# roatienza/efficientspeech

Measured on AMD Instinct MI355X. Metric: mel-frames/sec (whole node), full Phoneme2Mel forward, higher is better.
Workload: dtype f32 (weight GEMMs: fp32 operands split into 2 f16 pieces (22 significand bits, weights pre-scaled 2^8), 3 f16-MFMA products, fp32 accumulate)

## Files before the change

efficientspeech_amd/csrc/esmi_dev.h:

```cpp
#pragma once
#include "wavesim_shim.h"

namespace esmi {

__device__ __forceinline__ bf16x3 split_bf16x3(const f32x4& x0, const f32x4& x1) {
    unsigned h[8], m[8], l[8];
#pragma unroll
    for (int j = 0; j < 8; ++j) {
        const float x = j < 4 ? x0[j & 3] : x1[j & 3];
        h[j] = __builtin_bit_cast(unsigned, x) & 0xFFFF0000u;
        const float r1 = x - __builtin_bit_cast(float, h[j]);
        m[j] = __builtin_bit_cast(unsigned, r1) & 0xFFFF0000u;
        const float r2 = r1 - __builtin_bit_cast(float, m[j]);
        l[j] = __builtin_bit_cast(unsigned, r2);
    }
    bf16x3 o;
#pragma unroll
    for (int j = 0; j < 4; ++j) {
        o.hi[j] = pack_hi16(h[2 * j], h[2 * j + 1]);
        o.mid[j] = pack_hi16(m[2 * j], m[2 * j + 1]);
        o.lo[j] = pack_hi16(l[2 * j], l[2 * j + 1]);
    }
    return o;
}
__device__ __forceinline__ f32x16 mfma32_split(const bf16x3& a, const u32x4& bh, const u32x4& bm, const u32x4& bl, f32x16 c) {
    c = mfma32_bf16(a.hi, bh, c);
    c = mfma32_bf16(a.hi, bm, c);
    c = mfma32_bf16(a.mid, bh, c);
    c = mfma32_bf16(a.mid, bm, c);
    c = mfma32_bf16(a.hi, bl, c);
    c = mfma32_bf16(a.lo, bh, c);
    return c;
}
__device__ __forceinline__ f32x16 mfma32_split_wx(const u32x4& bh, const u32x4& bm, const u32x4& bl, const bf16x3& a, f32x16 c) {
    c = mfma32_bf16(bh, a.hi, c);
    c = mfma32_bf16(bm, a.hi, c);
    c = mfma32_bf16(bh, a.mid, c);
    c = mfma32_bf16(bm, a.mid, c);
    c = mfma32_bf16(bl, a.hi, c);
    c = mfma32_bf16(bh, a.lo, c);
    return c;
}

__device__ __forceinline__ f16x2p split_f16x2(const f32x4& x0, const f32x4& x1) {
    f16x2p o;
#pragma unroll
    for (int j = 0; j < 4; ++j) {
        const float a = j < 2 ? x0[2 * j] : x1[2 * j - 4], b = j < 2 ? x0[2 * j + 1] : x1[2 * j - 3];
        unsigned h1, h2;
        split_f16_pair(a, b, h1, h2);
        o.h1[j] = h1;
        o.h2[j] = h2;
    }
    return o;
}
__device__ __forceinline__ f32x16 mfma32_split2(const f16x2p& a, const u32x4& b1, const u32x4& b2, f32x16 c) {
    c = mfma32_f16(a.h2, b1, c);
    c = mfma32_f16(a.h1, b2, c);
    c = mfma32_f16(a.h1, b1, c);
    return c;
}
__device__ __forceinline__ f32x16 mfma32_split2_wx(const u32x4& b1, const u32x4& b2, const f16x2p& a, f32x16 c) {
    c = mfma32_f16(b1, a.h2, c);
    c = mfma32_f16(b2, a.h1, c);
    c = mfma32_f16(b1, a.h1, c);
    return c;
}

__device__ __forceinline__ float row_sum32(float v) {
    v += dpp_f<0xB1>(v);
    v += dpp_f<0x4E>(v);
    v += dpp_f<0x141>(v);
    v += dpp_f<0x140>(v);
    v += swz_xor16_f(v);
    return v;
}
__device__ __forceinline__ float row_sum16(float v) {
    v += dpp_f<0xB1>(v);
    v += dpp_f<0x4E>(v);
    v += dpp_f<0x141>(v);
    v += dpp_f<0x140>(v);
    return v;
}
template <int N>
__device__ __forceinline__ float row_sum_n(float v) {
    v += dpp_f<0xB1>(v);
    v += dpp_f<0x4E>(v);
    if (N >= 8) v += dpp_f<0x141>(v);
    if (N >= 16) v += dpp_f<0x140>(v);
    return v;
}
__device__ __forceinline__ float row_max32(float v) {
    v = fmaxf(v, dpp_f<0xB1>(v));
    v = fmaxf(v, dpp_f<0x4E>(v));
    v = fmaxf(v, dpp_f<0x141>(v));
    v = fmaxf(v, dpp_f<0x140>(v));
    v = fmaxf(v, swz_xor16_f(v));
    return v;
}

__device__ __forceinline__ float gelu_fast_f32(float x) {
    const float z = fabsf(x) * 0.70710678118654752440f;
    const float t = rcp_fast_f32(fmaf(0.3275911f, z, 1.0f));
    float pl = fmaf(1.061405429f, t, -1.453152027f);
    pl = fmaf(pl, t, 1.421413741f);
    pl = fmaf(pl, t, -0.284496736f);
    pl = fmaf(pl, t, 0.254829592f);
    const float erf_abs = 1.0f - pl * t * exp_fast_f32(-z * z);
    return 0.5f * x * (1.0f + copysignf(erf_abs, x));
}
__device__ __forceinline__ float ident_f32(float x) { return x; }
__device__ __forceinline__ float gelu_erf_f32(float x) {
    return 0.5f * x * (1.0f + erff(x * 0.70710678118654752440f));
}
enum Act { ACT_NONE = 0, ACT_RELU = 1, ACT_GELU = 2, ACT_TANH = 3 };
__device__ __forceinline__ float apply_act(float v, int act) {
    switch (act) {
        case ACT_RELU: return fmaxf(v, 0.0f);
        case ACT_GELU: return gelu_erf_f32(v);
        case ACT_TANH: return tanh_f32(v);
        default: return v;
    }
}

template <int NT>
__device__ __forceinline__ void layernorm_tile(f32x16 (&v)[NT], const float* __restrict__ g,
                                               const float* __restrict__ b, int lane, float eps = 1e-5f) {
    const float inv_c = 1.0f / (float)(32 * NT);
    float gg[NT], bb[NT];
#pragma unroll
    for (int nt = 0; nt < NT; ++nt) {
        gg[nt] = g[32 * nt + (lane & 31)];
        bb[nt] = b[32 * nt + (lane & 31)];
    }
#pragma unroll
    for (int r = 0; r < 16; ++r) {
        float s = 0.0f;
#pragma unroll
        for (int nt = 0; nt < NT; ++nt) s += v[nt][r];
        const float mean = row_sum32(s) * inv_c;
        float q = 0.0f;
#pragma unroll
        for (int nt = 0; nt < NT; ++nt) {
            const float d = v[nt][r] - mean;
            q = fmaf(d, d, q);
        }
        const float var = row_sum32(q) * inv_c;
        const float rstd = 1.0f / sqrtf(var + eps);
// ... 49 lines not shown
```

efficientspeech_amd/csrc/mel_decoder.h:

```cpp
#pragma once
#include <type_traits>

#include "dec_layout.h"

namespace esmi {

constexpr int kDecWps128 = 4, kDecWeightRing256 = 2;

__device__ __forceinline__ int batch_max_len(const int* __restrict__ mel_len, int B) {
    const int lane = lane_id();
    int v = 0;
    for (int j = lane; j < B; j += 64) v = max(v, mel_len[j]);
    float f = row_max32((float)v);
    f = fmaxf(f, swap32_f(f));
    return uniform_i((int)f);
}

template <int DX2, int NV>
__device__ __forceinline__ void dec_ln_regs(f32x4 (&v)[NV], const f32x4 (&g)[NV], const f32x4 (&be)[NV]) {
    float s = 0.0f;
#pragma unroll
    for (int k = 0; k < NV; ++k) s += (v[k][0] + v[k][1]) + (v[k][2] + v[k][3]);
    s = row_sum_n<16>(s);
    const float mean = s * (1.0f / DX2);
    float q = 0.0f;
#pragma unroll
    for (int k = 0; k < NV; ++k) {
#pragma unroll
        for (int e = 0; e < 4; ++e) {
            v[k][e] -= mean;
            q = fmaf(v[k][e], v[k][e], q);
        }
    }
    q = row_sum_n<16>(q);
    const float rstd = rsqrt_fast_f32(q * (1.0f / DX2) + 1e-5f);
#pragma unroll
    for (int k = 0; k < NV; ++k) {
#pragma unroll
        for (int e = 0; e < 4; ++e) v[k][e] = fmaf(v[k][e] * rstd, g[k][e], be[k][e]);
    }
}
template <int NV>
__device__ __forceinline__ void dec_owner_ld(const float* pv, f32x4 (&o)[NV]) {
#pragma unroll
    for (int k = 0; k < NV; ++k) o[k] = *reinterpret_cast<const f32x4*>(pv + 4 * 16 * k);
}
template <int DX2>
__device__ __forceinline__ void dec_store_planes(unsigned* base, int off, const f32x4& v) {
    typedef unsigned u32x2 __attribute__((ext_vector_type(2)));
    unsigned h1a, h2a, h1b, h2b;
    split_f16_pair(v[0], v[1], h1a, h2a);
    split_f16_pair(v[2], v[3], h1b, h2b);
    unsigned* rowp = base + off;
    *reinterpret_cast<u32x2*>(rowp) = u32x2{h1a, h1b};
    *reinterpret_cast<u32x2*>(rowp + DX2 / 2) = u32x2{h2a, h2b};
}

__device__ __forceinline__ void dec_store_plane16(unsigned* base, int off, const f32x4& v) {
    typedef unsigned u32x2 __attribute__((ext_vector_type(2)));
    *reinterpret_cast<u32x2*>(base + off) = u32x2{round_f16_pair(v[0], v[1]), round_f16_pair(v[2], v[3])};
}

__device__ __forceinline__ void dec_store_plane_bf16(unsigned* base, int off, const f32x4& v) {
    typedef unsigned u32x2 __attribute__((ext_vector_type(2)));
    *reinterpret_cast<u32x2*>(base + off) = u32x2{round_bf16_pair(v[0], v[1]), round_bf16_pair(v[2], v[3])};
}

__device__ __forceinline__ void dec_clk_stamp(int ck_) {
    long long* const clk = g_dec_clk;
    if (clk && threadIdx.x == 0) {
        if (blockIdx.x == 0) {
            const int slot = ck_ == 0 ? 0 : 1;
            clk[2 * slot] = clock_shader();
            clk[2 * slot + 1] = clock_real100();
        }
    }
}
template <int MT, int NTW>
__device__ __forceinline__ void dec_zero_acc(f32x16 (&acc)[MT][NTW]) {
#pragma unroll
    for (int mt = 0; mt < MT; ++mt) {
#pragma unroll
        for (int t = 0; t < NTW; ++t) acc[mt][t] = zero16();
    }
}

using DecPrecisionMode = PrecisionMode;
constexpr PrecisionMode DEC_PM_SPLIT = PM_SPLIT, DEC_PM_F16 = PM_F16, DEC_PM_BF16 = PM_BF16;
template <int DX2, int KD, int NW, bool HALF16 = false>
__global__ __launch_bounds__(64 * NW, (DX2 <= 128 ? kDecWps128 : NW / 4)) void mel_decoder_kernel(const MelDecP p) {
    constexpr int PM = HALF16 ? DEC_PM_F16 : DEC_PM_SPLIT;
#include "mel_decoder_body.h"
}
template <int DX2, int KD, int NW>
__global__ __launch_bounds__(64 * NW, (DX2 <= 128 ? kDecWps128 : NW / 4)) void mel_decoder_bf16_kernel(const MelDecP p) {
    constexpr int PM = DEC_PM_BF16;
#include "mel_decoder_body.h"
}

template <int DX2, int KD, PrecisionMode PM>
int set_dec_clock(long long* slots) { return store_dec_clock_pointer(slots); }

template <int DX2, int KD, PrecisionMode PM>
int launch_mel_decoder(const MelDecP& p, dim3 grid, hipStream_t st) {
    if constexpr (precision_mode_built(PM)) {
        constexpr int NW = 8;
        const int lds = (dec_lds_floats<DX2>(KD) + p.carry_lds_layers * (KD / 2) * DX2) * (int)sizeof(float);
        if constexpr (PM == PM_SPLIT) {
            ESMI_LAUNCH_LDS((mel_decoder_kernel<DX2, KD, NW>), grid, dim3(64 * NW), lds, st, p);
        } else if constexpr (PM == PM_F16) {
            ESMI_LAUNCH_LDS((mel_decoder_kernel<DX2, KD, NW, true>), grid, dim3(64 * NW), lds, st, p);
        } else {
            ESMI_LAUNCH_LDS((mel_decoder_bf16_kernel<DX2, KD, NW>), grid, dim3(64 * NW), lds, st, p);
        }
        return launch_status();
    }
    return ESMI_ERR_UNSUPPORTED;
}

}

#define ESMI_DEC_INSTANCE(DX2, KD, PM)                                                                \
    ESMI_TU_RANGE_SETTER(dec_##DX2##_##KD##_##PM)                                                     \
    namespace esmi {                                                                                  \
    template int set_dec_clock<DX2, KD, PM>(long long*);                                              \
    template int launch_mel_decoder<DX2, KD, PM>(const MelDecP&, dim3, hipStream_t);                  \
    }
```

efficientspeech_amd/csrc/mel_decoder_body.h:

```cpp
    constexpr bool P16 = PM == DEC_PM_F16, BF = PM == DEC_PM_BF16, ONE = P16 || BF;
    static_assert(!ONE || ESMI_DEC_SPLIT == 2, "precision 16 and bf16 exist in the split build only");
    constexpr int NPL = ONE ? 1 : 2;
    constexpr int NPLR = P16 ? 1 : 2;
    constexpr int kDecThreads = 64 * NW;
    constexpr int NS = 4;
    constexpr int MH = NW / NS;
    constexpr int MT = 4 / MH;
    constexpr int TPR = 16;
    constexpr int RPT = kDecRows * TPR / kDecThreads;
    constexpr int NTW = DX2 / (32 * NS);
    constexpr int WCOLS = 32 * NTW;
    constexpr int KCH = DX2 / 128;
    constexpr int LDSROW = DX2 + 4;
    constexpr bool SPLIT = ESMI_DEC_SPLIT == 2;
    constexpr float WSI = SPLIT && !BF ? kF16WScaleInv : 1.0f;
    constexpr int PAD = KD / 2;
    constexpr int CG = DX2 / 4;
    constexpr int RS = kDecRows / (kDecThreads / CG);
    constexpr int NV = DX2 / (4 * TPR);
    constexpr bool STREAM = DX2 > 128;
    constexpr bool LNA = DX2 > 128;
    ESMI_DYN_LDS(lds);
    constexpr int PB = (KD + 6) * DX2;
    constexpr int P_DWB = KD * DX2, P_PWB = P_DWB + DX2, P_G = P_PWB + DX2, P_B = P_G + DX2, P_SG = P_B + DX2,
                  P_SB = P_SG + DX2;
    constexpr int NA4 = (KD + 1) * DX2 / 4;
    constexpr int NB4 = 3 * DX2 / 4;
    static_assert(NA4 <= kDecThreads && NB4 + DX2 / 2 <= kDecThreads, "param staging: one float4 per thread per group");
    float* xs = lds;
    float* pbuf = lds + (kDecRows + 2 * kDecPadRows) * LDSROW;
    int* src = reinterpret_cast<int*>(pbuf + PB);

    int tid = (int)threadIdx.x, lane = lane_id();
    const int w = uniform_i(wave_id());
    int i = lane & 31, h = lane >> 5;
    const int mh = w / NS, ns = w % NS;
    int seg, b;
    {
        const int id = (int)blockIdx.x, per8 = 8 * p.n_seg;
        const int g = id / per8, r = id - g * per8;
        seg = r >> 3;
        b = 8 * g + (r & 7);
        if (b >= p.B) return;
    }
    const int L = p.lmax_dev ? *p.lmax_dev : (p.lmax_host >= 0 ? p.lmax_host : batch_max_len(p.mel_len, p.B));
    const int mlen = p.mel_len ? min(p.mel_len[b], L) : L;
    const int valid_end = p.apply_mask ? mlen : L;
    const int s0 = seg * p.seg_len, s1 = min(s0 + p.seg_len, p.L_out);
    if (s0 >= p.L_out) return;
    int f0 = 0, g0 = 0, f_lo = 0, out_hi = 0;
    const int n_layers = p.n_blocks * p.block_depth;
    const DecLay<DX2, KD> lay(p.d4, p.n_blocks, p.block_depth);
    const BufRsrc brs = make_rsrc(p.blob, (long)lay.total * (long)sizeof(float));
    unsigned tid16 = (unsigned)tid * 16u, lane16 = (unsigned)lane * 16u;
    auto blob_ld = [&](int float_off, unsigned voff) __attribute__((always_inline)) { return buf_ld4s(brs, voff, (unsigned)(float_off * 4)); };
#ifdef ESMI_DEC_TRACE
    int tr_n = 0;
    const bool tr_on = p.trace && seg == (DX2 > 128 ? 0 : 3) && b == p.B / 2 + 5 && lane == 0;
#define ESMI_STAMP() do { if (tr_on && tr_n < 59) p.trace[w * 64 + tr_n] = (long long)__builtin_amdgcn_s_memtime(); ++tr_n; } while (0)
#define ESMI_STAMP_AT(slot) do { if (tr_on && ck == 0) p.trace[w * 64 + (slot)] = (long long)__builtin_amdgcn_s_memtime(); } while (0)
    if (tr_on) p.trace[w * 64 + 62] = clock_real100();
    ESMI_STAMP();
#else
#define ESMI_STAMP() do {} while (0)
#endif

    auto stage = [&](int float_off, float* dst, int n4) __attribute__((always_inline)) {
        if (tid < n4) lds_dma16(p.blob + float_off + opaque_i(4 * tid), dst + 256 * w, lane);
    };
    auto fetch_A = [&](int l) __attribute__((always_inline)) {
        if (l < n_layers) stage(lay.layer0 + l * lay.layer_stride, pbuf, NA4);
    };
    auto fetch_B = [&](int l) __attribute__((always_inline)) {
        if (l < n_layers) {
            stage(lay.layer0 + l * lay.layer_stride + lay.l_pwb, pbuf + P_PWB, NB4);
            if (((l + 1) % p.block_depth) == 0) {
                if (tid >= NB4 && tid < NB4 + DX2 / 2)
                    lds_dma16(p.blob + (lay.skip0 + (l / p.block_depth) * 2 * DX2) + opaque_i(4 * (tid - NB4)), pbuf + P_PWB + 256 * w, lane);
            }
        } else {
            stage(lay.mel_b, pbuf, DX2 / 4);
        }
    };

    float* const cws = STREAM && p.carry_ws ? p.carry_ws + ((long)seg * p.B + b) * p.ws_stride : nullptr;
    float* const stat = reinterpret_cast<float*>(src + kDecRows);
    float* const cbuf = stat + (LNA ? 2 * kDecRows * NS * 2 : 0);
    float cnext = 0.0f;
    const bool skew = STREAM && cws && p.skew;
    const DecWalk wk(skew, PAD, p.n_blocks, p.block_depth, p.halo);
    const int sh = wk.sh, off_last = wk.lead();
    const int bc_n4 = (sh + PAD) * CG;
    float* const bcw = skew ? cws + n_layers * (PAD * DX2) : nullptr;
    const int hl0 = s0 > 0 ? wk.lost() : off_last;
    const int keep = wk.keep();
    bool edge_window = false;
    int fb_cur = 0;
    auto lane_refresh = [&]() __attribute__((always_inline)) {
        tid = opaque_i(tid);
        lane = tid & 63; i = lane & 31; h = lane >> 5;
        tid16 = (unsigned)tid * 16u; lane16 = (unsigned)lane * 16u;
    };
    if constexpr (!STREAM) dec_clk_stamp(0);
    for (int ck = 0;; ++ck) {
    if constexpr (STREAM) lane_refresh();
    if constexpr (STREAM) dec_clk_stamp(ck);
    g0 = s0 - hl0 + ck * keep;
    f0 = g0 + off_last;
    f_lo = max(g0, s0);
    if ((!(STREAM && cws) && ck > 0) || f_lo >= s1) break;
    out_hi = min(g0 + keep, s1);
    if (f_lo >= valid_end) {
        const int n = (s1 - f_lo) * p.n_mel;
        float* o = p.mel + ((long)b * p.L_out + f_lo) * p.n_mel;
        for (int e = tid; e < n; e += kDecThreads) o[e] = 0.0f;
        break;
    }
    if (ck > 0) __syncthreads();
// ... 3 lines not shown
            if (slot >= 0 && cws && ck > 0 && tid < PAD * DX2) {
                if (slot < p.carry_lds_layers) cnext = cbuf[slot * (PAD * DX2) + tid];
                else cnext = cws[slot * (PAD * DX2) + opaque_i(tid)];
            }
        }
    };
    auto carry_put = [&](int slot) __attribute__((always_inline)) {
        if constexpr (STREAM) {
            if (slot >= 0 && tid < PAD * DX2) xs[(kDecPadRows - PAD + tid / DX2) * LDSROW + tid % DX2] = cnext;
        }
    };
    auto carry_save = [&](int slot) __attribute__((always_inline)) {
        if constexpr (STREAM) {
            if (slot >= 0 && cws && tid < PAD * DX2) {
                const float v = xs[(kDecPadRows + keep - PAD + tid / DX2) * LDSROW + tid % DX2];
                if (slot < p.carry_lds_layers) cbuf[slot * (PAD * DX2) + tid] = v;
                else cws[slot * (PAD * DX2) + opaque_i(tid)] = v;
            }
        }
    };
    int* const cum_s = reinterpret_cast<int*>(xs + kDecPadRows * LDSROW);
    const bool cum_lds = p.cum && p.T <= kDecRows * LDSROW;
    if (cum_lds) {
        const int* crow = p.cum + b * p.T;
        for (int e = tid; e < p.T; e += kDecThreads) cum_s[e] = crow[e];
    }
    for (int e = tid; e < 2 * kDecPadRows * LDSROW; e += kDecThreads) {
        const int r = e / LDSROW, c = e - r * LDSROW;
        const int rr = r < kDecPadRows ? r : kDecRows + r;
        xs[rr * LDSROW + c] = 0.0f;
    }
    if (tid < NB4)
        reinterpret_cast<f32x4*>(pbuf + P_PWB)[tid] = blob_ld(lay.proj_b, tid16);
    carry_load(0);
    fetch_A(0);
#ifdef ESMI_DEC_TRACE
    ESMI_STAMP_AT(52);
#endif
    if (cum_lds) __syncthreads();
#ifdef ESMI_DEC_TRACE
    ESMI_STAMP_AT(53);
#endif
    if (tid < kDecRows) {
        const int f = f0 + tid;
        int s;
        if (f < 0 || f >= L) s = -1;
        else if (p.cum) {
            if (f < mlen) {
                int ph;
                if (cum_lds) {
                    int lo = 0, hi = p.T;
                    while (lo < hi) {
                        const int mid = (lo + hi) >> 1;
                        if (cum_s[mid] > f) hi = mid;
                        else lo = mid + 1;
                    }
                    ph = lo;
                } else ph = frame_to_phoneme(p.cum + b * p.T, p.T, f);
                s = ph < p.T ? b * p.T + ph : -2;
            } else s = -2;
        } else s = b * L + f;
        src[tid] = s;
    }
    __syncthreads();
    ESMI_STAMP();

    constexpr int LNPER = 16 / RPT;
    int ln_c = lane & (TPR - 1), ln_row0 = 64 * (w / LNPER) + 16 * (lane / TPR) + RPT * (w % LNPER);
    auto owner_ptr = [&]() __attribute__((always_inline)) { return xs + opaque_i((kDecPadRows + ln_row0) * LDSROW + 4 * ln_c); };
    auto owner_load = [&](f32x4 (&v)[RPT][NV], const float* ln_ptr) __attribute__((always_inline)) {
#pragma unroll
        for (int j = 0; j < RPT; ++j) {
#pragma unroll
            for (int k = 0; k < NV; ++k) v[j][k] = *reinterpret_cast<const f32x4*>(ln_ptr + j * LDSROW + 4 * TPR * k);
        }
    };
    auto set_edge = [&](int fbase) __attribute__((always_inline)) {
        edge_window = fbase < 0 || fbase + kDecRows > L;
        fb_cur = fbase;
    };
    auto row_inside = [&](int j) __attribute__((always_inline)) { return (unsigned)(fb_cur + ln_row0 + j) < (unsigned)L; };
    set_edge(f0);
    f32x16 acc[MT][NTW];
    f32x16 skipA[LNA ? MT : 1][LNA ? NTW : 1];
    f32x4 skip[RPT][NV];
#pragma unroll
    for (int j = 0; j < RPT; ++j) {
#pragma unroll
        for (int v = 0; v < NV; ++v) skip[j][v] = zero4();
    }

    constexpr int KSUB = DX2 <= 128 ? (SPLIT ? 4 : 8) / NTW : (NW > 8 ? 2 : 8);
    constexpr int KS16 = KSUB / 2;
    std::conditional_t<SPLIT, u32x4[NTW][KS16][NPL], f32x4[NTW][KSUB]> bf;
    auto load_b = [&](int wsl, int k0) __attribute__((always_inline)) {
        if constexpr (SPLIT) {
#pragma unroll
            for (int t = 0; t < NTW; ++t) {
#pragma unroll
                for (int st = 0; st < KS16; ++st) {
                    if constexpr (BF) {
                        const int o = wsl + ((t * 8 + (k0 >> 1) + st) * 2) * 256;
                        bf[t][st][0] = bf16_of_f16_planes(__builtin_bit_cast(u32x4, blob_ld(o, lane16)), __builtin_bit_cast(u32x4, blob_ld(o + 256, lane16)));
                    } else {
#pragma unroll
                        for (int pl = 0; pl < NPL; ++pl)
                            bf[t][st][pl] = __builtin_bit_cast(u32x4, blob_ld(wsl + ((t * 8 + (k0 >> 1) + st) * 2 + pl) * 256, lane16));
                    }
                }
            }
        } else {
#pragma unroll
            for (int t = 0; t < NTW; ++t) {
#pragma unroll
                for (int kc = 0; kc < KSUB; ++kc) bf[t][kc] = blob_ld(wsl + (t * 16 + k0 + kc) * 256, lane16);
            }
        }
    };
    auto mma_sub = [&](int a_col0, int k0) __attribute__((always_inline)) {
        if constexpr (SPLIT) {
            const float* a_base = xs + opaque_i((kDecPadRows + 32 * MT * mh + i) * LDSROW + 8 * h);
#pragma unroll
            for (int st = 0; st < KS16; ++st) {
#pragma unroll
                for (int mt = 0; mt < MT; ++mt) {
                    const float* ap = a_base + 32 * mt * LDSROW + a_col0 + 8 * k0 + 16 * st;
                    if constexpr (BF) {
                        const u32x4 a1 = round_bf16x8(*reinterpret_cast<const f32x4*>(ap), *reinterpret_cast<const f32x4*>(ap + 4));
#pragma unroll
                        for (int t = 0; t < NTW; ++t) acc[mt][t] = mfma32_bf16(bf[t][st][0], a1, acc[mt][t]);
                    } else if constexpr (P16) {
                        const u32x4 a1 = round_f16x8(*reinterpret_cast<const f32x4*>(ap), *reinterpret_cast<const f32x4*>(ap + 4));
#pragma unroll
                        for (int t = 0; t < NTW; ++t) acc[mt][t] = mfma32_f16(bf[t][st][0], a1, acc[mt][t]);
                    } else {
                        const f16x2p a2 = split_f16x2(*reinterpret_cast<const f32x4*>(ap), *reinterpret_cast<const f32x4*>(ap + 4));
#pragma unroll
                        for (int t = 0; t < NTW; ++t) acc[mt][t] = mfma32_split2_wx(bf[t][st][0], bf[t][st][1], a2, acc[mt][t]);
                    }
                }
            }
        } else {
            const float* a_base = xs + opaque_i((kDecPadRows + 32 * MT * mh + i) * LDSROW + 4 * h);
#pragma unroll
            for (int mt = 0; mt < MT; ++mt) {
#pragma unroll
                for (int kc = 0; kc < KSUB; ++kc) {
                    const f32x4 av = *reinterpret_cast<const f32x4*>(a_base + 32 * mt * LDSROW + a_col0 + 8 * (k0 + kc));
#pragma unroll
                    for (int s = 0; s < 4; ++s) {
#pragma unroll
                        for (int t = 0; t < NTW; ++t) acc[mt][t] = mfma32(bf[t][kc][s], av[s], acc[mt][t]);
                    }
                }
            }
        }
    };
    auto wslice = [&](int off, int c) __attribute__((always_inline)) { return off + (c * (DX2 / 32) + ns * NTW) * 16 * 256; };

    constexpr int WD = DX2 > 128 ? kDecWeightRing256 : 0;
    constexpr int NSTEP = 8 * KCH, NITEM = NSTEP * MT;
    static_assert(WD >= 0 && WD <= NSTEP, "ring depth");
    u32x4 wr[WD > 0 ? WD : 1][NTW][NPLR];
    auto w_fetch = [&](int off, int s, int slot, auto ntc) __attribute__((always_inline)) {
        constexpr int NT = decltype(ntc)::value;
        const int wsl = off + ((s >> 3) * (4 * NT) + ns * NT) * 8 * 2 * 256;
#pragma unroll
        for (int t = 0; t < NT; ++t) {
#pragma unroll
            for (int pl = 0; pl < NPLR; ++pl) wr[slot][t][pl] = __builtin_bit_cast(u32x4, blob_ld(wsl + ((t * 8 + (s & 7)) * 2 + pl) * 256, lane16));
        }
    };
    auto gemm_prefetch = [&](int off, auto ntc) __attribute__((always_inline)) {
        if constexpr (SPLIT && WD > 0) {
#pragma unroll
            for (int s = 0; s < WD; ++s) w_fetch(off, s, s, ntc);
            sched_fence();
        }
    };
    auto gemm_planes = [&](int off, auto ntc) __attribute__((always_inline)) {
        constexpr int NT = decltype(ntc)::value;
        static_assert(WD > 0 || NT == NTW, "the un-pipelined form keeps the layers' slice width");
        const unsigned* a_base = reinterpret_cast<const unsigned*>(xs) + opaque_i((kDecPadRows + 32 * MT * mh + i) * LDSROW + 4 * h);
        if constexpr (WD == 0) {
#pragma unroll
            for (int c = 0; c < KCH; ++c) {
#pragma unroll
                for (int k0 = 0; k0 < 16; k0 += KSUB) {
                    load_b(wslice(off, c), k0);
#pragma unroll
                    for (int st = 0; st < KS16; ++st) {
#pragma unroll
                        for (int mt = 0; mt < MT; ++mt) {
                            const unsigned* ap = a_base + 32 * mt * LDSROW + 64 * c + 4 * k0 + 8 * st;
                            if constexpr (BF) {
                                const u32x4 a1 = *reinterpret_cast<const u32x4*>(ap);
#pragma unroll
                                for (int t = 0; t < NTW; ++t) acc[mt][t] = mfma32_bf16(bf[t][st][0], a1, acc[mt][t]);
                            } else if constexpr (P16) {
                                const u32x4 a1 = *reinterpret_cast<const u32x4*>(ap);
#pragma unroll
                                for (int t = 0; t < NTW; ++t) acc[mt][t] = mfma32_f16(bf[t][st][0], a1, acc[mt][t]);
                            } else {
                                f16x2p a2;
                                a2.h1 = *reinterpret_cast<const u32x4*>(ap);
                                a2.h2 = *reinterpret_cast<const u32x4*>(ap + DX2 / 2);
#pragma unroll
                                for (int t = 0; t < NTW; ++t) acc[mt][t] = mfma32_split2_wx(bf[t][st][0], bf[t][st][1], a2, acc[mt][t]);
                            }
                        }
                    }
                }
            }
        } else {
            f16x2p ar;
            [[maybe_unused]] u32x4 wc[NT];
            auto a_fetch = [&](int q) __attribute__((always_inline)) {
                const int s = q / MT, mt = q % MT;
                const unsigned* ap = a_base + 32 * mt * LDSROW + 64 * (s >> 3) + 8 * (s & 7);
                ar.h1 = *reinterpret_cast<const u32x4*>(ap);
                if constexpr (!ONE) ar.h2 = *reinterpret_cast<const u32x4*>(ap + DX2 / 2);
            };
            a_fetch(0);
            sched_fence();
#pragma unroll
            for (int q = 0; q < NITEM; ++q) {
                const int s = q / MT, mt = q % MT;
                if constexpr (BF) {
                    if (mt == 0) {
#pragma unroll
                        for (int t = 0; t < NT; ++t) wc[t] = bf16_of_f16_planes(wr[s % (WD > 0 ? WD : 1)][t][0], wr[s % (WD > 0 ? WD : 1)][t][1]);
                    }
                }
#pragma unroll
                for (int t = 0; t < NT; ++t) {
                    if constexpr (BF) acc[mt][t] = mfma32_bf16(wc[t], ar.h1, acc[mt][t]);
                    else if constexpr (P16) acc[mt][t] = mfma32_f16(wr[s % (WD > 0 ? WD : 1)][t][0], ar.h1, acc[mt][t]);
                    else acc[mt][t] = mfma32_split2_wx(wr[s % (WD > 0 ? WD : 1)][t][0], wr[s % (WD > 0 ? WD : 1)][t][1], ar, acc[mt][t]);
                }
                if (q + 1 < NITEM) a_fetch(q + 1);
                if (mt == MT - 1 && s + WD < NSTEP) w_fetch(off, s + WD, s % (WD > 0 ? WD : 1), ntc);
                sched_fence();
            }
        }
    };
    auto gemm_rows = [&](int off) __attribute__((always_inline)) {
#pragma unroll
        for (int c = 0; c < KCH; ++c) {
#pragma unroll
            for (int k0 = 0; k0 < 16; k0 += KSUB) {
                load_b(wslice(off, c), k0);
                mma_sub(128 * c, k0);
            }
        }
    };

    auto acc_col = [&](int t) __attribute__((always_inline)) { return ns * WCOLS + 32 * t + 4 * h; };
    auto tanh_acc = [&](const float* bias) __attribute__((always_inline)) {
#pragma unroll
        for (int t = 0; t < NTW; ++t) {
            const float* bp = bias + opaque_i(acc_col(t));
#pragma unroll
            for (int g = 0; g < 4; ++g) {
                const f32x4 bc = *reinterpret_cast<const f32x4*>(bp + 8 * g) * kTanhExpScale;
#pragma unroll
                for (int mt = 0; mt < MT; ++mt) {
#pragma unroll
                    for (int e = 0; e < 4; ++e) acc[mt][t][4 * g + e] = tanh_fast_fma_f32(acc[mt][t][4 * g + e], WSI * kTanhExpScale, bc[e]);
                }
            }
        }
    };
    auto store_acc = [&]() __attribute__((always_inline)) {
#pragma unroll
        for (int t = 0; t < NTW; ++t) {
            float* base = xs + opaque_i((kDecPadRows + 32 * MT * mh + i) * LDSROW + ns * WCOLS + 32 * t + 4 * h);
#pragma unroll
            for (int g = 0; g < 4; ++g) {
#pragma unroll
                for (int mt = 0; mt < MT; ++mt) {
                    f32x4 v;
#pragma unroll
                    for (int e = 0; e < 4; ++e) v[e] = acc[mt][t][4 * g + e];
                    *reinterpret_cast<f32x4*>(base + 32 * mt * LDSROW + 8 * g) = v;
                }
            }
        }
    };
    auto stats_put = [&](int buf) __attribute__((always_inline)) {
        typedef float f32x2 __attribute__((ext_vector_type(2)));
#pragma unroll
        for (int mt = 0; mt < MT; ++mt) {
            float s1 = 0.0f, m2 = 0.0f;
#pragma unroll
            for (int t = 0; t < NTW; ++t) {
#pragma unroll
                for (int r = 0; r < 16; ++r) s1 += acc[mt][t][r];
            }
            s1 += swap32_f(s1);
            const float lmean = s1 * (1.0f / WCOLS);
#pragma unroll
            for (int t = 0; t < NTW; ++t) {
#pragma unroll
                for (int r = 0; r < 16; ++r) {
                    const float d = acc[mt][t][r] - lmean;
                    m2 = fmaf(d, d, m2);
                }
            }
            m2 += swap32_f(m2);
            if (h == 0) *reinterpret_cast<f32x2*>(stat + opaque_i(((buf * kDecRows + 32 * MT * mh + i) * NS + ns) * 2) + 32 * mt * NS * 2) = f32x2{s1, m2};
        }
    };
    auto stats_get = [&](int buf, float (&mean)[MT], float (&rstd)[MT]) __attribute__((always_inline)) {
        const float* sp = stat + opaque_i((buf * kDecRows + 32 * MT * mh + i) * NS * 2);
#pragma unroll
        for (int mt = 0; mt < MT; ++mt) {
            const f32x4 a = *reinterpret_cast<const f32x4*>(sp + 32 * mt * NS * 2), b = *reinterpret_cast<const f32x4*>(sp + 32 * mt * NS * 2 + 4);
            const float s1 = (a[0] + a[2]) + (b[0] + b[2]);
            mean[mt] = s1 * (1.0f / DX2);
            const float d0 = fmaf(a[0], 1.0f / WCOLS, -mean[mt]), d1 = fmaf(a[2], 1.0f / WCOLS, -mean[mt]);
            const float d2 = fmaf(b[0], 1.0f / WCOLS, -mean[mt]), d3 = fmaf(b[2], 1.0f / WCOLS, -mean[mt]);
            const float m2 = fmaf((float)WCOLS, fmaf(d0, d0, d1 * d1) + fmaf(d2, d2, d3 * d3), (a[1] + a[3]) + (b[1] + b[3]));
            rstd[mt] = rsqrt_fast_f32(m2 * (1.0f / DX2) + 1e-5f);
        }
    };
    auto ln_acc = [&](const float* gain, const float* shift, const float (&mean)[MT], const float (&rstd)[MT]) __attribute__((always_inline)) {
#pragma unroll
        for (int t = 0; t < NTW; ++t) {
            const float* gp = gain + opaque_i(acc_col(t));
            const float* bp = shift + opaque_i(acc_col(t));
#pragma unroll
            for (int g = 0; g < 4; ++g) {
                const f32x4 gv = *reinterpret_cast<const f32x4*>(gp + 8 * g), bv = *reinterpret_cast<const f32x4*>(bp + 8 * g);
#pragma unroll
                for (int mt = 0; mt < MT; ++mt) {
#pragma unroll
                    for (int e = 0; e < 4; ++e) acc[mt][t][4 * g + e] = fmaf((acc[mt][t][4 * g + e] - mean[mt]) * rstd[mt], gv[e], bv[e]);
                }
            }
        }
    };
    auto store_ln = [&](bool planes_, int shw) __attribute__((always_inline)) {
        bool inside[MT], keep_row[MT];
#pragma unroll
        for (int mt = 0; mt < MT; ++mt) {
            const int row = 32 * MT * mh + 32 * mt + i;
            inside[mt] = !edge_window || (unsigned)(fb_cur + row) < (unsigned)L;
            keep_row[mt] = row + shw < kDecRows;
        }
#pragma unroll
        for (int t = 0; t < NTW; ++t) {
            float* base = xs + opaque_i((kDecPadRows + 32 * MT * mh + i + shw) * LDSROW + ns * WCOLS + 32 * t + 4 * h);
            unsigned* pbase = reinterpret_cast<unsigned*>(xs) + opaque_i((kDecPadRows + 32 * MT * mh + i) * LDSROW + acc_col(t) / 2);
#pragma unroll
            for (int g = 0; g < 4; ++g) {
#pragma unroll
                for (int mt = 0; mt < MT; ++mt) {
                    f32x4 v;
#pragma unroll
                    for (int e = 0; e < 4; ++e) v[e] = inside[mt] ? acc[mt][t][4 * g + e] : 0.0f;
                    if (SPLIT && planes_) {
                        if constexpr (BF) dec_store_plane_bf16(pbase, 32 * mt * LDSROW + 4 * g, v);
                        else if constexpr (P16) dec_store_plane16(pbase, 32 * mt * LDSROW + 4 * g, v);
                        else dec_store_planes<DX2>(pbase, 32 * mt * LDSROW + 4 * g, v);
                    } else if (keep_row[mt]) {
                        *reinterpret_cast<f32x4*>(base + 32 * mt * LDSROW + 8 * g) = v;
                    }
                }
            }
        }
    };
    auto ln_pass = [&](const float* pb0, bool block_end_, bool planes_, int shw) __attribute__((always_inline)) {
        const float* pb = pb0 + opaque_i(4 * ln_c);
        float* ln_ptr = owner_ptr();
        f32x4 g[NV], be[NV];
        dec_owner_ld(pb + P_G, g);
        dec_owner_ld(pb + P_B, be);
        f32x4 v[RPT][NV];
        owner_load(v, ln_ptr);
#pragma unroll
        for (int j = 0; j < RPT; ++j) dec_ln_regs<DX2>(v[j], g, be);
        if (block_end_) {
            dec_owner_ld(pb + P_SG, g);
            dec_owner_ld(pb + P_SB, be);
#pragma unroll
            for (int j = 0; j < RPT; ++j) {
#pragma unroll
                for (int k = 0; k < NV; ++k) v[j][k] += skip[j][k];
                dec_ln_regs<DX2>(v[j], g, be);
            }
        }
        if (edge_window) {
#pragma unroll
            for (int j = 0; j < RPT; ++j) {
#pragma unroll
                for (int k = 0; k < NV; ++k)
                    if (!row_inside(j)) v[j][k] = zero4();
            }
        }
        if (SPLIT && planes_) {
#pragma unroll
            for (int j = 0; j < RPT; ++j) {
#pragma unroll
                for (int k = 0; k < NV; ++k) {
                    if constexpr (BF) {
                        dec_store_plane_bf16(reinterpret_cast<unsigned*>(ln_ptr + j * LDSROW) - 2 * ln_c, 2 * TPR * k, v[j][k]);
                    } else if constexpr (P16) {
                        dec_store_plane16(reinterpret_cast<unsigned*>(ln_ptr + j * LDSROW) - 2 * ln_c, 2 * TPR * k, v[j][k]);
                    } else {
                        typedef unsigned u32x2 __attribute__((ext_vector_type(2)));
                        unsigned h1a, h2a, h1b, h2b;
                        split_f16_pair(v[j][k][0], v[j][k][1], h1a, h2a);
                        split_f16_pair(v[j][k][2], v[j][k][3], h1b, h2b);
                        unsigned* rowp = reinterpret_cast<unsigned*>(ln_ptr + j * LDSROW) - 2 * ln_c + 2 * TPR * k;
                        *reinterpret_cast<u32x2*>(rowp) = u32x2{h1a, h1b};
                        *reinterpret_cast<u32x2*>(rowp + DX2 / 2) = u32x2{h2a, h2b};
                    }
                }
            }
            return;
        }
        float* wp = ln_ptr;
        if (STREAM && shw) {
            __syncthreads();
            wp = ln_ptr + shw * LDSROW;
        }
#pragma unroll
        for (int j = 0; j < RPT; ++j) {
            if (STREAM && ln_row0 + j + shw >= kDecRows) continue;
#pragma unroll
            for (int k = 0; k < NV; ++k) *reinterpret_cast<f32x4*>(wp + j * LDSROW + 4 * TPR * k) = v[j][k];
        }
    };
    typedef std::true_type TrueC;
    typedef std::false_type FalseC;
    constexpr int NTM = (SPLIT && DX2 > 128) ? 1 : NTW;
    typedef std::integral_constant<int, NTW> NtwC;
    typedef std::integral_constant<int, NTM> NtmC;

    if (p.h0) {
        static_assert(kDecRows * (DX2 / 4) % kDecThreads == 0, "whole passes");
        for (int it = 0; it < kDecRows * (DX2 / 4) / kDecThreads; ++it) {
            const int e = tid + it * kDecThreads;
            const int r = e / (DX2 / 4), q = e - r * (DX2 / 4);
            const int s = src[r];
            f32x4 v = zero4();
            if (s >= 0) v = STREAM ? __builtin_nontemporal_load(reinterpret_cast<const f32x4*>(p.h0 + (long)s * DX2 + 4 * q)) : ld4(p.h0 + (long)s * DX2 + 4 * q);
            else if (s == -2) {
                const f32x4 bb = *reinterpret_cast<const f32x4*>(pbuf + P_PWB + 4 * q);
#pragma unroll
                for (int c = 0; c < 4; ++c) v[c] = tanh_fast_f32(bb[c]);
            }
            *reinterpret_cast<f32x4*>(xs + (kDecPadRows + r) * LDSROW + 4 * q) = v;
        }
#ifdef ESMI_DEC_TRACE
        ESMI_STAMP_AT(54);
#endif
        __syncthreads();
#ifdef ESMI_DEC_TRACE
        ESMI_STAMP_AT(55);
#endif
        {
            const float* pb = pbuf + opaque_i(4 * ln_c);
            float* ln_ptr = owner_ptr();
            owner_load(skip, ln_ptr);
            unsigned pad_rows = 0;
#pragma unroll
            for (int j = 0; j < RPT; ++j) pad_rows |= (src[ln_row0 + j] == -2 ? 1u : 0u) << j;
            if (ballot64(pad_rows != 0u) != 0ull) {
                f32x4 g[NV], be[NV];
                dec_owner_ld(pb + P_G, g);
                dec_owner_ld(pb + P_B, be);
#pragma unroll
                for (int j = 0; j < RPT; ++j) {
                    f32x4 u[NV];
#pragma unroll
                    for (int k = 0; k < NV; ++k) u[k] = skip[j][k];
                    dec_ln_regs<DX2>(u, g, be);
#pragma unroll
                    for (int k = 0; k < NV; ++k) {
                        if ((pad_rows >> j) & 1u) skip[j][k] = u[k];
                        *reinterpret_cast<f32x4*>(ln_ptr + j * LDSROW + 4 * TPR * k) = skip[j][k];
                    }
                }
            }
        }
        carry_put(0);
        __syncthreads();
    } else {
        dec_zero_acc(acc);
        const int nchunks = p.d4 / 128;
        for (int ch = 0; ch < nchunks; ++ch) {
            if (ch > 0) __syncthreads();
            for (int e = tid; e < kDecRows * 32; e += kDecThreads) {
                const int r = e >> 5, q = e & 31;
                const int s = src[r];
                f32x4 v = zero4();
                if (s >= 0) v = ld4(p.x + (long)s * p.d4 + ch * 128 + 4 * q);
                *reinterpret_cast<f32x4*>(xs + (kDecPadRows + r) * LDSROW + 4 * q) = v;
            }
            __syncthreads();
#pragma unroll
            for (int k0 = 0; k0 < 16; k0 += KSUB) {
                load_b(wslice(0, ch), k0);
                mma_sub(0, k0);
            }
        }
        tanh_acc(pbuf + P_PWB);
        __syncthreads();
        store_acc();
        __syncthreads();
        {
            const float* pb = pbuf + opaque_i(4 * ln_c);
            float* ln_ptr = owner_ptr();
            f32x4 g[NV], be[NV];
            dec_owner_ld(pb + P_G, g);
            dec_owner_ld(pb + P_B, be);
#pragma unroll
            for (int j = 0; j < RPT; ++j) {
#pragma unroll
                for (int k = 0; k < NV; ++k) skip[j][k] = *reinterpret_cast<const f32x4*>(ln_ptr + j * LDSROW + 4 * TPR * k);
                dec_ln_regs<DX2>(skip[j], g, be);
#pragma unroll
                for (int k = 0; k < NV; ++k) {
                    if (!row_inside(j)) skip[j][k] = zero4();
                    *reinterpret_cast<f32x4*>(ln_ptr + j * LDSROW + 4 * TPR * k) = skip[j][k];
                }
            }
        }
        carry_put(0);
        __syncthreads();
    }

    ESMI_STAMP();
    int dw_cg = tid % CG, dw_r0 = (tid / CG) * RS;
    int blk = 0, lin = 0;
    for (int l = 0; l < n_layers; ++l) {
        const float* pb = pbuf;
        const int lbase = lay.layer0 + l * lay.layer_stride;
        const bool block_end = lin + 1 == p.block_depth;
        const int slot = skew ? ((lin == 0 && l > 0) ? -1 : l - blk) : l;
        const int slot_next = skew ? (block_end ? -1 : l + 1 - blk) : l + 1;
        if constexpr (STREAM) {
            lane_refresh();
            ln_c = lane & (TPR - 1); ln_row0 = 64 * (w / LNPER) + 16 * (lane / TPR) + RPT * (w % LNPER);
            dw_cg = tid % CG; dw_r0 = (tid / CG) * RS;
            if (skew && lin == 0 && l > 0) {
                if (tid < bc_n4) {
                    const f32x4 v = *reinterpret_cast<const f32x4*>(xs + (kDecPadRows + keep - PAD + tid / CG) * LDSROW + 4 * (tid % CG));
                    *reinterpret_cast<f32x4*>(bcw + (blk - 1) * (4 * kDecBlockCarry4) + opaque_i(4 * tid)) = v;
                }
                set_edge(g0 + sh * (p.n_blocks - 1 - blk));
            }
        }
        if constexpr (LNA) {
            if (lin == 0) {
#pragma unroll
                for (int t = 0; t < NTW; ++t) {
                    const float* base = xs + opaque_i((kDecPadRows + 32 * MT * mh + i) * LDSROW + ns * WCOLS + 32 * t + 4 * h);
#pragma unroll
                    for (int g = 0; g < 4; ++g) {
#pragma unroll
                        for (int mt = 0; mt < MT; ++mt) {
                            const f32x4 v = *reinterpret_cast<const f32x4*>(base + 32 * mt * LDSROW + 8 * g);
#pragma unroll
                            for (int e = 0; e < 4; ++e) skipA[mt][t][4 * g + e] = v[e];
                        }
                    }
                }
            }
        }
        if (!LNA && lin == 0 && l > 0) {
            const float* ln_ptr = owner_ptr();
            owner_load(skip, ln_ptr);
        }
        ESMI_STAMP();
        {
            f32x4 win[RS + 2 * PAD];
            float* col = xs + opaque_i((kDecPadRows + dw_r0 - PAD) * LDSROW + 4 * dw_cg);
            const float* pbt = pb + opaque_i(4 * dw_cg);
            unsigned* prow = reinterpret_cast<unsigned*>(xs) + opaque_i((kDecPadRows + dw_r0) * LDSROW + 2 * dw_cg);
            fetch_B(l);
#pragma unroll
            for (int r = 0; r < RS + 2 * PAD; ++r) win[r] = *reinterpret_cast<const f32x4*>(col + r * LDSROW);
            f32x4 tap[KD];
#pragma unroll
            for (int j = 0; j < KD; ++j) tap[j] = *reinterpret_cast<const f32x4*>(pbt + j * DX2);
            const f32x4 tb = *reinterpret_cast<const f32x4*>(pbt + P_DWB);
            carry_save(slot);
            ESMI_STAMP();
            __syncthreads();
            ESMI_STAMP();
#pragma unroll
            for (int r = 0; r < RS; ++r) {
                f32x4 a = tb;
#pragma unroll
                for (int j = 0; j < KD; ++j) {
#pragma unroll
                    for (int e = 0; e < 4; ++e) a[e] = fmaf(win[r + j][e], tap[j][e], a[e]);
                }
                if (SPLIT) {
                    if constexpr (BF) dec_store_plane_bf16(prow, r * LDSROW, a);
                    else if constexpr (P16) dec_store_plane16(prow, r * LDSROW, a);
                    else dec_store_planes<DX2>(prow, r * LDSROW, a);
                } else {
                    *reinterpret_cast<f32x4*>(col + (r + PAD) * LDSROW) = a;
                }
            }
        }
        gemm_prefetch(lbase + lay.l_pw, NtwC{});
        ESMI_STAMP();
        __syncthreads();
        ESMI_STAMP();
        dec_zero_acc(acc);
        if constexpr (SPLIT) gemm_planes(lbase + lay.l_pw, NtwC{});
        else gemm_rows(lbase + lay.l_pw);
        ESMI_STAMP();
        tanh_acc(pb + P_PWB);
        if constexpr (LNA) stats_put(0);
        fetch_A(l + 1);
        ESMI_STAMP();
        __syncthreads();
        ESMI_STAMP();
        if constexpr (!LNA) store_acc();
        ESMI_STAMP();
        if constexpr (!LNA) __syncthreads();
        ESMI_STAMP();
        if (l + 1 == n_layers) fetch_B(n_layers);
        else carry_load(slot_next);
        const int shw = (STREAM && skew && block_end && l + 1 < n_layers) ? sh : 0;
        if constexpr (LNA) {
            float mean[MT], rstd[MT];
            stats_get(0, mean, rstd);
            ln_acc(pb + P_G, pb + P_B, mean, rstd);
            if (block_end) {
#pragma unroll
                for (int mt = 0; mt < MT; ++mt) {
#pragma unroll
                    for (int t = 0; t < NTW; ++t) acc[mt][t] += skipA[mt][t];
                }
                stats_put(1);
                __syncthreads();
                stats_get(1, mean, rstd);
                ln_acc(pb + P_SG, pb + P_SB, mean, rstd);
            }
            store_ln(SPLIT && l + 1 == n_layers, shw);
        } else {
            ln_pass(pb, block_end, SPLIT && l + 1 == n_layers, shw);
        }
        ESMI_STAMP();
        if (l + 1 == n_layers) gemm_prefetch(lay.mel_w, NtmC{});
        else carry_put(slot_next);
        if constexpr (STREAM) {
            if (shw && tid < bc_n4) {
                f32x4 bcv = zero4();
                if (ck > 0) bcv = ld4(bcw + blk * (4 * kDecBlockCarry4) + opaque_i(4 * tid));
                *reinterpret_cast<f32x4*>(xs + (kDecPadRows - PAD + tid / CG) * LDSROW + 4 * (tid % CG)) = bcv;
            }
        }
        __syncthreads();
        ESMI_STAMP();
        if (++lin == p.block_depth) { lin = 0; ++blk; }
    }

#ifdef ESMI_DEC_TRACE
    ESMI_STAMP_AT(59);
#endif
    if constexpr (!STREAM) {
        long long* const clk = g_dec_clk;
        if (clk && blockIdx.x == 0 && w == 0) {
            typedef long long i64x2 __attribute__((ext_vector_type(2)));
            *reinterpret_cast<i64x2*>(clk + 2) = i64x2{clock_shader(), clock_real100()};
        }
    }
    if (n_layers == 0) {
        fetch_B(0);
        __syncthreads();
    }
    const bool mel_wave = ns * 32 * NTM < p.n_mel;
    const float* mb = pbuf;
    const bool vec_ok = (p.n_mel & 3) == 0;
    if (mel_wave) {
        dec_zero_acc(acc);
        if constexpr (SPLIT) {
            if (n_layers > 0) gemm_planes(lay.mel_w, NtmC{});
            else gemm_rows(lay.mel_w);
        } else {
            gemm_rows(lay.mel_w);
        }
    }
#ifdef ESMI_DEC_TRACE
    ESMI_STAMP_AT(60);
#endif
    if constexpr (STREAM) {
        float* stg = xs;
        const int mstride = (p.n_mel + 3) & ~3;
        __syncthreads();
        if (mel_wave) {
#pragma unroll
            for (int t = 0; t < NTM; ++t) {
#pragma unroll
                for (int mt = 0; mt < MT; ++mt) {
                    const int r = 32 * MT * mh + 32 * mt + i;
                    const bool live = g0 + r < valid_end;
#pragma unroll
                    for (int g = 0; g < 4; ++g) {
                        const int col = ns * 32 * NTM + 32 * t + 8 * g + 4 * h;
                        if (col >= p.n_mel) continue;
                        const f32x4 bc = *reinterpret_cast<const f32x4*>(mb + col);
                        f32x4 v;
#pragma unroll
                        for (int e = 0; e < 4; ++e) v[e] = live ? fmaf(acc[mt][t][4 * g + e], WSI, bc[e]) : 0.0f;
                        *reinterpret_cast<f32x4*>(stg + r * mstride + col) = v;
                    }
                }
            }
        }
        __syncthreads();
        const float* sp = stg + (f_lo - g0) * mstride;
        float* dp = p.mel + ((long)b * p.L_out + f_lo) * p.n_mel;
        if (vec_ok) {
            const int n4 = (out_hi - f_lo) * (p.n_mel >> 2);
            for (int e = tid; e < n4; e += kDecThreads) {
                __builtin_nontemporal_store(*reinterpret_cast<const f32x4*>(sp + 4 * e), reinterpret_cast<f32x4*>(dp + 4 * e));
            }
        } else {
            const int n = (out_hi - f_lo) * p.n_mel;
            for (int e = tid; e < n; e += kDecThreads) dp[e] = sp[(e / p.n_mel) * mstride + e % p.n_mel];
        }
    } else if (mel_wave) {
#pragma unroll
        for (int t = 0; t < NTM; ++t) {
#pragma unroll
            for (int mt = 0; mt < MT; ++mt) {
                const int f = g0 + 32 * MT * mh + 32 * mt + i;
                if (f < f_lo || f >= out_hi) continue;
                float* orow = p.mel + ((long)b * p.L_out + f) * p.n_mel;
                const bool live = f < valid_end;
#pragma unroll
                for (int g = 0; g < 4; ++g) {
                    const int col = ns * 32 * NTM + 32 * t + 8 * g + 4 * h;
                    if (col >= p.n_mel) continue;
                    const f32x4 bc = *reinterpret_cast<const f32x4*>(mb + col);
                    f32x4 v;
#pragma unroll
                    for (int e = 0; e < 4; ++e) v[e] = live ? fmaf(acc[mt][t][4 * g + e], WSI, bc[e]) : 0.0f;
                    if (vec_ok) {
                        *reinterpret_cast<f32x4*>(orow + col) = v;
                    } else {
#pragma unroll
                        for (int e = 0; e < 4; ++e)
                            if (col + e < p.n_mel) orow[col + e] = v[e];
                    }
                }
            }
        }
    }
#ifdef ESMI_DEC_TRACE
    ESMI_STAMP_AT(61);
    if (tr_on && ck == 0) p.trace[w * 64 + 63] = clock_real100();
#endif
    }
```

Before: 882.6 million.

## Use 16x16 MFMA tiles for decoder pointwise and mel GEMMs

Adds a 16-row MFMA path (mfma16 with f32x4 accumulators) to the mel decoder for the DX2<=128 split case. The 64-frame x 32-channel wave tile is covered by 4x2 16x16 tiles instead of 32x32 tiles, with new weight-lane indexing, accumulator store, tanh epilogue and mel output writes. The mel GEMM can skip the second column tile when it falls past n_mel. This changes the MFMA shape, register footprint and LDS access pattern, and the new lane indexing carries a correctness risk.

```diff
diff --git a/efficientspeech_amd/csrc/esmi_dev.h b/efficientspeech_amd/csrc/esmi_dev.h
--- a/efficientspeech_amd/csrc/esmi_dev.h
+++ b/efficientspeech_amd/csrc/esmi_dev.h
@@ -64,6 +64,12 @@
     c = mfma32_f16(b1, a.h2, c);
     c = mfma32_f16(b2, a.h1, c);
     c = mfma32_f16(b1, a.h1, c);
+    return c;
+}
+__device__ __forceinline__ f32x4 mfma16_split2_wx(const u32x4& b1, const u32x4& b2, const f16x2p& a, f32x4 c) {
+    c = mfma16_f16(b1, a.h2, c);
+    c = mfma16_f16(b2, a.h1, c);
+    c = mfma16_f16(b1, a.h1, c);
     return c;
 }
 
diff --git a/efficientspeech_amd/csrc/mel_decoder.h b/efficientspeech_amd/csrc/mel_decoder.h
--- a/efficientspeech_amd/csrc/mel_decoder.h
+++ b/efficientspeech_amd/csrc/mel_decoder.h
@@ -2,6 +2,10 @@
 #include <type_traits>
 
 #include "dec_layout.h"
+
+#ifndef ESMI_DEC_MFMA16
+#define ESMI_DEC_MFMA16 1
+#endif
 
 namespace esmi {
 
@@ -84,6 +88,14 @@
         for (int t = 0; t < NTW; ++t) acc[mt][t] = zero16();
     }
 }
+template <int RT, int CT>
+__device__ __forceinline__ void dec_zero_acc(f32x4 (&acc)[RT][CT]) {
+#pragma unroll
+    for (int rt = 0; rt < RT; ++rt) {
+#pragma unroll
+        for (int ct = 0; ct < CT; ++ct) acc[rt][ct] = zero4();
+    }
+}
 
 using DecPrecisionMode = PrecisionMode;
 constexpr PrecisionMode DEC_PM_SPLIT = PM_SPLIT, DEC_PM_F16 = PM_F16, DEC_PM_BF16 = PM_BF16;
diff --git a/efficientspeech_amd/csrc/mel_decoder_body.h b/efficientspeech_amd/csrc/mel_decoder_body.h
--- a/efficientspeech_amd/csrc/mel_decoder_body.h
+++ b/efficientspeech_amd/csrc/mel_decoder_body.h
@@ -20,6 +20,8 @@
     constexpr int NV = DX2 / (4 * TPR);
     constexpr bool STREAM = DX2 > 128;
     constexpr bool LNA = DX2 > 128;
+    constexpr bool M16 = SPLIT && DX2 <= 128 && ((ESMI_DEC_MFMA16 >> (P16 ? 1 : BF ? 2 : 0)) & 1) != 0;
+    static_assert(!M16 || (MT == 2 && NTW == 1 && KCH == 1), "the 16-row form is written for the 64-frame x 32-channel wave tile");
     ESMI_DYN_LDS(lds);
     constexpr int PB = (KD + 6) * DX2;
     constexpr int P_DWB = KD * DX2, P_PWB = P_DWB + DX2, P_G = P_PWB + DX2, P_B = P_G + DX2, P_SG = P_B + DX2,
@@ -34,6 +36,7 @@
     int tid = (int)threadIdx.x, lane = lane_id();
     const int w = uniform_i(wave_id());
     int i = lane & 31, h = lane >> 5;
+    [[maybe_unused]] const int j16 = lane & 15, g16 = lane >> 4;
     const int mh = w / NS, ns = w % NS;
     int seg, b;
     {
@@ -203,6 +206,9 @@
     auto row_inside = [&](int j) __attribute__((always_inline)) { return (unsigned)(fb_cur + ln_row0 + j) < (unsigned)L; };
     set_edge(f0);
     f32x16 acc[MT][NTW];
+    f32x4 acc4[M16 ? 2 * MT : 1][M16 ? 2 * NTW : 1];
+    [[maybe_unused]] auto acc_row = [&](int rt) __attribute__((always_inline)) { return 32 * MT * mh + 16 * rt + j16; };
+    [[maybe_unused]] auto acc_col16 = [&](int ct) __attribute__((always_inline)) { return ns * WCOLS + 16 * ct + 4 * g16; };
     f32x16 skipA[LNA ? MT : 1][LNA ? NTW : 1];
     f32x4 skip[RPT][NV];
 #pragma unroll
@@ -214,8 +220,28 @@
     constexpr int KSUB = DX2 <= 128 ? (SPLIT ? 4 : 8) / NTW : (NW > 8 ? 2 : 8);
     constexpr int KS16 = KSUB / 2;
     std::conditional_t<SPLIT, u32x4[NTW][KS16][NPL], f32x4[NTW][KSUB]> bf;
+    [[maybe_unused]] auto wlane16 = [&]() __attribute__((always_inline)) {
+        return (unsigned)opaque_i((j16 + 32 * (g16 & 1)) * 16 + (g16 >> 1) * (2 * 256 * 4));
+    };
+    [[maybe_unused]] auto load_b16 = [&](int wsl, int S, unsigned wl16, auto nctc) __attribute__((always_inline)) {
+        if constexpr (M16) {
+            constexpr int NCT = decltype(nctc)::value;
+#pragma unroll
+            for (int ct = 0; ct < NCT; ++ct) {
+                const int o = wsl + (2 * S * 2) * 256;
+                if constexpr (BF) {
+                    bf[0][ct][0] = bf16_of_f16_planes(__builtin_bit_cast(u32x4, blob_ld(o, wl16 + 256u * ct)), __builtin_bit_cast(u32x4, blob_ld(o + 256, wl16 + 256u * ct)));
+                } else {
+#pragma unroll
+                    for (int pl = 0; pl < NPL; ++pl) bf[0][ct][pl] = __builtin_bit_cast(u32x4, blob_ld(o + pl * 256, wl16 + 256u * ct));
+                }
+            }
+        }
+    };
     auto load_b = [&](int wsl, int k0) __attribute__((always_inline)) {
-        if constexpr (SPLIT) {
+        if constexpr (M16) {
+            load_b16(wsl, k0 >> 2, wlane16(), std::integral_constant<int, 2>{});
+        } else if constexpr (SPLIT) {
 #pragma unroll
             for (int t = 0; t < NTW; ++t) {
 #pragma unroll
@@ -239,7 +265,27 @@
         }
     };
     auto mma_sub = [&](int a_col0, int k0) __attribute__((always_inline)) {
-        if constexpr (SPLIT) {
+        if constexpr (M16) {
+            static_assert(!M16 || (KSUB == 4 && KS16 == 2), "a weight sub-slice is one 32-channel step");
+            const float* a_base = xs + opaque_i((kDecPadRows + 32 * MT * mh + j16) * LDSROW + 8 * g16);
+#pragma unroll
+            for (int rt = 0; rt < 2 * MT; ++rt) {
+                const float* ap = a_base + 16 * rt * LDSROW + a_col0 + 8 * k0;
+                if constexpr (BF) {
+                    const u32x4 a1 = round_bf16x8(*reinterpret_cast<const f32x4*>(ap), *reinterpret_cast<const f32x4*>(ap + 4));
+#pragma unroll
+                    for (int ct = 0; ct < 2; ++ct) acc4[rt][ct] = mfma16_bf16(bf[0][ct][0], a1, acc4[rt][ct]);
+                } else if constexpr (P16) {
+                    const u32x4 a1 = round_f16x8(*reinterpret_cast<const f32x4*>(ap), *reinterpret_cast<const f32x4*>(ap + 4));
+#pragma unroll
+                    for (int ct = 0; ct < 2; ++ct) acc4[rt][ct] = mfma16_f16(bf[0][ct][0], a1, acc4[rt][ct]);
+                } else {
+                    const f16x2p a2 = split_f16x2(*reinterpret_cast<const f32x4*>(ap), *reinterpret_cast<const f32x4*>(ap + 4));
+#pragma unroll
+                    for (int ct = 0; ct < 2; ++ct) acc4[rt][ct] = mfma16_split2_wx(bf[0][ct][0], bf[0][ct][1], a2, acc4[rt][ct]);
+                }
+            }
+        } else if constexpr (SPLIT) {
             const float* a_base = xs + opaque_i((kDecPadRows + 32 * MT * mh + i) * LDSROW + 8 * h);
 #pragma unroll
             for (int st = 0; st < KS16; ++st) {
@@ -365,6 +411,37 @@
             }
         }
     };
+    [[maybe_unused]] auto gemm_planes16 = [&](int off, auto nctc) __attribute__((always_inline)) {
+        if constexpr (M16) {
+            constexpr int NCT = decltype(nctc)::value;
+            const unsigned* a_base = reinterpret_cast<const unsigned*>(xs) + opaque_i((kDecPadRows + 32 * MT * mh + j16) * LDSROW + 4 * g16);
+            const unsigned wl16 = wlane16();
+#pragma unroll
+            for (int S = 0; S < DX2 / 32; ++S) {
+                load_b16(wslice(off, 0), S, wl16, nctc);
+                if constexpr (BF) sched_fence();
+#pragma unroll
+                for (int rt = 0; rt < 2 * MT; ++rt) {
+                    const unsigned* ap = a_base + 16 * rt * LDSROW + 16 * S;
+                    if constexpr (BF) {
+                        const u32x4 a1 = *reinterpret_cast<const u32x4*>(ap);
+#pragma unroll
+                        for (int ct = 0; ct < NCT; ++ct) acc4[rt][ct] = mfma16_bf16(bf[0][ct][0], a1, acc4[rt][ct]);
+                    } else if constexpr (P16) {
+                        const u32x4 a1 = *reinterpret_cast<const u32x4*>(ap);
+#pragma unroll
+                        for (int ct = 0; ct < NCT; ++ct) acc4[rt][ct] = mfma16_f16(bf[0][ct][0], a1, acc4[rt][ct]);
+                    } else {
+                        f16x2p a2;
+                        a2.h1 = *reinterpret_cast<const u32x4*>(ap);
+                        a2.h2 = *reinterpret_cast<const u32x4*>(ap + DX2 / 2);
+#pragma unroll
+                        for (int ct = 0; ct < NCT; ++ct) acc4[rt][ct] = mfma16_split2_wx(bf[0][ct][0], bf[0][ct][1], a2, acc4[rt][ct]);
+                    }
+                }
+            }
+        }
+    };
     auto gemm_rows = [&](int off) __attribute__((always_inline)) {
 #pragma unroll
         for (int c = 0; c < KCH; ++c) {
@@ -378,6 +455,18 @@
 
     auto acc_col = [&](int t) __attribute__((always_inline)) { return ns * WCOLS + 32 * t + 4 * h; };
     auto tanh_acc = [&](const float* bias) __attribute__((always_inline)) {
+        if constexpr (M16) {
+#pragma unroll
+            for (int ct = 0; ct < 2 * NTW; ++ct) {
+                const f32x4 bc = *reinterpret_cast<const f32x4*>(bias + opaque_i(acc_col16(ct))) * kTanhExpScale;
+#pragma unroll
+                for (int rt = 0; rt < 2 * MT; ++rt) {
+#pragma unroll
+                    for (int e = 0; e < 4; ++e) acc4[rt][ct][e] = tanh_fast_fma_f32(acc4[rt][ct][e], WSI * kTanhExpScale, bc[e]);
+                }
+            }
+            return;
+        }
 #pragma unroll
         for (int t = 0; t < NTW; ++t) {
             const float* bp = bias + opaque_i(acc_col(t));
@@ -393,6 +482,15 @@
         }
     };
     auto store_acc = [&]() __attribute__((always_inline)) {
+        if constexpr (M16) {
+            float* base = xs + opaque_i((kDecPadRows + acc_row(0)) * LDSROW + acc_col16(0));
+#pragma unroll
+            for (int ct = 0; ct < 2 * NTW; ++ct) {
+#pragma unroll
+                for (int rt = 0; rt < 2 * MT; ++rt) *reinterpret_cast<f32x4*>(base + 16 * rt * LDSROW + 16 * ct) = acc4[rt][ct];
+            }
+            return;
+        }
 #pragma unroll
         for (int t = 0; t < NTW; ++t) {
             float* base = xs + opaque_i((kDecPadRows + 32 * MT * mh + i) * LDSROW + ns * WCOLS + 32 * t + 4 * h);
@@ -558,6 +656,8 @@
     constexpr int NTM = (SPLIT && DX2 > 128) ? 1 : NTW;
     typedef std::integral_constant<int, NTW> NtwC;
     typedef std::integral_constant<int, NTM> NtmC;
+    typedef std::integral_constant<int, 1> OneC;
+    typedef std::integral_constant<int, 2> TwoC;
 
     if (p.h0) {
         static_assert(kDecRows * (DX2 / 4) % kDecThreads == 0, "whole passes");
@@ -609,7 +709,8 @@
         carry_put(0);
         __syncthreads();
     } else {
-        dec_zero_acc(acc);
+        if constexpr (M16) dec_zero_acc(acc4);
+        else dec_zero_acc(acc);
         const int nchunks = p.d4 / 128;
         for (int ch = 0; ch < nchunks; ++ch) {
             if (ch > 0) __syncthreads();
@@ -733,8 +834,10 @@
         ESMI_STAMP();
         __syncthreads();
         ESMI_STAMP();
-        dec_zero_acc(acc);
-        if constexpr (SPLIT) gemm_planes(lbase + lay.l_pw, NtwC{});
+        if constexpr (M16) dec_zero_acc(acc4);
+        else dec_zero_acc(acc);
+        if constexpr (M16) gemm_planes16(lbase + lay.l_pw, TwoC{});
+        else if constexpr (SPLIT) gemm_planes(lbase + lay.l_pw, NtwC{});
         else gemm_rows(lbase + lay.l_pw);
         ESMI_STAMP();
         tanh_acc(pb + P_PWB);
@@ -802,8 +905,13 @@
     const float* mb = pbuf;
     const bool vec_ok = (p.n_mel & 3) == 0;
     if (mel_wave) {
-        dec_zero_acc(acc);
-        if constexpr (SPLIT) {
+        if constexpr (M16) dec_zero_acc(acc4);
+        else dec_zero_acc(acc);
+        if constexpr (M16) {
+            if (n_layers == 0) gemm_rows(lay.mel_w);
+            else if (ns * WCOLS + 16 < p.n_mel) gemm_planes16(lay.mel_w, TwoC{});
+            else gemm_planes16(lay.mel_w, OneC{});
+        } else if constexpr (SPLIT) {
             if (n_layers > 0) gemm_planes(lay.mel_w, NtmC{});
             else gemm_rows(lay.mel_w);
         } else {
@@ -849,6 +957,32 @@
             const int n = (out_hi - f_lo) * p.n_mel;
             for (int e = tid; e < n; e += kDecThreads) dp[e] = sp[(e / p.n_mel) * mstride + e % p.n_mel];
         }
+    } else if (M16 && mel_wave) {
+        if constexpr (M16) {
+#pragma unroll
+            for (int rt = 0; rt < 2 * MT; ++rt) {
+                const int f = g0 + acc_row(rt);
+                if (f < f_lo || f >= out_hi) continue;
+                float* orow = p.mel + ((long)b * p.L_out + f) * p.n_mel;
+                const bool live = f < valid_end;
+#pragma unroll
+                for (int ct = 0; ct < 2 * NTM; ++ct) {
+                    const int col = acc_col16(ct);
+                    if (col >= p.n_mel) continue;
+                    const f32x4 bc = *reinterpret_cast<const f32x4*>(mb + col);
+                    f32x4 v;
+#pragma unroll
+                    for (int e = 0; e < 4; ++e) v[e] = live ? fmaf(acc4[rt][ct][e], WSI, bc[e]) : 0.0f;
+                    if (vec_ok) {
+                        *reinterpret_cast<f32x4*>(orow + col) = v;
+                    } else {
+#pragma unroll
+                        for (int e = 0; e < 4; ++e)
+                            if (col + e < p.n_mel) orow[col + e] = v[e];
+                    }
+                }
+            }
+        }
     } else if (mel_wave) {
 #pragma unroll
         for (int t = 0; t < NTM; ++t) {
```

Result: faster. 920.0 million, median of 6 (+4.2%).
